# geopolars/geopolars

Measured on AMD Instinct MI355X. Metric: predicate evals/sec (10M pts x 1k polys point-in-polygon), higher is better.
Workload: dtype f64

## Files before the change

geopolars_amd/_abi.py:

```python
from __future__ import annotations

import ctypes as C
import os

HERE = os.path.dirname(os.path.abspath(__file__))
LIB_PATH = os.environ.get("GPK_LIB_PATH") or os.path.join(HERE, "libgeopolars_hip.so")

GPK_OK = 0
GPK_ERR_MISMATCHED_GEOMETRY = 1
GPK_ERR_INVALID_OFFSETS = 2
GPK_ERR_NULL_UNSUPPORTED = 3
GPK_ERR_DEVICE = 4
GPK_ERR_OOM = 5
GPK_ERR_INVALID_ARGUMENT = 6
GPK_ERR_CAPACITY = 7

GEOM_POINT = 0
GEOM_LINESTRING = 1
GEOM_POLYGON = 3
GEOM_MULTIPOINT = 4
GEOM_MULTILINESTRING = 5
GEOM_MULTIPOLYGON = 6
ARROW_WKB, ARROW_INTERLEAVED, ARROW_STRUCT = 0, 1, 2

# ... 101 lines not shown
    "gpk_envelope": (C.c_int32, [_VP, _VP, _VP, C.c_int32, _VP]),
    "gpk_exterior": (C.c_int32, [_VP, _VP, _VP, C.POINTER(C.c_int64), C.c_int32, _VP]),
    "gpk_explode": (C.c_int32, [_VP, _VP, C.c_int32, _VP, C.POINTER(_VP)]),
    "gpk_geoarray_validity": (C.c_int32, [_VP, _VP, C.POINTER(C.c_int32), _VP]),
    "gpk_geoarray_len": (C.c_int32, [_VP, C.POINTER(C.c_int64)]),
    "gpk_geom_type": (C.c_int32, [_VP, _VP, C.c_int32, _VP]),
    "gpk_is_empty": (C.c_int32, [_VP, _VP, C.c_int32, _VP]),
    "gpk_is_ring": (C.c_int32, [_VP, _VP, C.c_int32, _VP]),
    "gpk_point_xy": (C.c_int32, [_VP, _VP, _VP, C.c_int32, _VP]),
    "gpk_geodesic_length": (C.c_int32, [_VP, C.c_int32, _VP, C.c_int32, _VP]),
    "gpk_simplify": (C.c_int32, [_VP, C.c_double, _VP, _VP, C.POINTER(C.c_int64), C.c_int32, _VP]),
    "gpk_convex_hull": (C.c_int32, [_VP, _VP, _VP, C.c_int32, _VP]),
    "gpk_distance_rowwise": (C.c_int32, [_VP, _VP, _VP, _VP, C.c_int32, _VP]),
    "gpk_rowmap_build": (C.c_int32, [_VP, _VP, C.c_int64, C.c_int32, _VP, C.POINTER(_VP)]),
    "gpk_rowmap_free": (C.c_int32, [_VP]),
    "gpk_rowmap_nbytes": (C.c_int32, [_VP, C.POINTER(C.c_int64)]),
    "gpk_distance_rowmap": (C.c_int32, [_VP, _VP, _VP, _VP, C.c_int32, _VP]),
    "gpk_predicate_rowwise": (C.c_int32, [_VP, _VP, _VP, C.c_int32, _VP, C.c_int32, _VP]),
    "gpk_index_build": (C.c_int32, [_VP, _VP, C.POINTER(_VP)]),
    "gpk_index_build_ex": (C.c_int32, [_VP, C.c_int32, _VP, _VP, C.POINTER(_VP)]),
    "gpk_index_free": (C.c_int32, [_VP]),
    "gpk_index_nbytes": (C.c_int32, [_VP, C.POINTER(C.c_int64)]),
    "gpk_index_describe": (C.c_int32, [_VP, C.POINTER(C.c_int64)]),
    "gpk_index_query_envelope": (C.c_int32, [_VP, _VP, C.c_int64, C.c_int32, _VP, _VP, C.c_int64, C.POINTER(C.c_int64), C.c_int32, _VP]),
    "gpk_spatial_join": (
        C.c_int32,
        [_VP, _VP, _VP, C.c_int32, C.c_uint32, _VP, _VP, C.c_int64, C.POINTER(C.c_int64), C.c_int32, _VP],
    ),
    "gpk_spatial_join_async": (C.c_int32, [_VP, _VP, _VP, C.c_int32, C.c_uint32, _VP, _VP, C.c_int64, _VP, _VP]),
    "gpk_nearest_join": (
        C.c_int32,
        [_VP, _VP, _VP, C.c_double, C.c_uint32, _VP, _VP, _VP, C.c_int64, C.POINTER(C.c_int64), C.c_int32, _VP],
    ),
    "gpk_dwithin_join": (
        C.c_int32,
        [_VP, _VP, _VP, C.c_double, C.c_uint32, _VP, _VP, _VP, C.c_int64, C.POINTER(C.c_int64), C.c_int32, _VP],
    ),
    "gpk_dwithin_rowwise": (C.c_int32, [_VP, _VP, _VP, C.c_double, _VP, C.c_int32, _VP]),
    "gpk_closest_point_rowwise": (C.c_int32, [_VP, _VP, _VP, _VP, _VP, C.c_int32, _VP]),
    "gpk_line_locate_point": (C.c_int32, [_VP, _VP, _VP, C.c_int32, _VP, C.c_int32, _VP]),
    "gpk_line_interpolate_point": (C.c_int32, [_VP, _VP, C.c_int64, C.c_int32, _VP, _VP, C.c_int32, _VP]),
    "gpk_wkb_encode": (C.c_int32, [_VP, _VP, _VP, C.c_int64, C.POINTER(C.c_int64)]),
    "gpk_geoarray_to_wkb": (C.c_int32, [_VP, _VP, _VP, C.c_int64, C.POINTER(C.c_int64), C.c_int32, _VP]),
    "gpk_join_indices": (C.c_int32, [_VP, _VP, C.c_int64, C.c_int64, C.c_uint32, C.c_int32, _VP, _VP, C.c_int64, C.POINTER(C.c_int64), C.c_int32, _VP]),
    "gpk_take_fixed": (C.c_int32, [_VP, C.c_int32, _VP, C.c_int64, _VP, C.c_int64, _VP, _VP, C.c_int32, _VP]),
    "gpk_take_binary": (C.c_int32, [_VP, _VP, _VP, C.c_int64, _VP, C.c_int64, _VP, _VP, C.c_int64, C.POINTER(C.c_int64), _VP, C.c_int32, _VP]),
# ... 73 lines not shown
```

geopolars_amd/csrc/gpk_gridindex.hip:

```cpp
#include <atomic>
#include <chrono>
#include <cmath>
#include <cstdlib>

#include "gpk_device.h"
#include "gpk_index.h"
#include "gpk_scan.h"

namespace gpk {

__global__ __launch_bounds__(256) void extent_partial_kernel(const double4* __restrict__ bbox, int64_t n, double4* __restrict__ part) {
    __shared__ double red[4][4];
    double mnx = INFINITY, mny = INFINITY, mxx = -INFINITY, mxy = -INFINITY;
    for (int64_t i = (int64_t)blockIdx.x * 256 + threadIdx.x; i < n; i += (int64_t)gridDim.x * 256) {
        const double4 b = bbox[i];
        if (b.x == b.x) {
            mnx = fmin(mnx, b.x);
            mny = fmin(mny, b.y);
            mxx = fmax(mxx, b.z);
            mxy = fmax(mxy, b.w);
        }
    }
    mnx = dev::wave_min(mnx);
    mny = dev::wave_min(mny);
// ... 108 lines not shown
extern "C" {

int32_t gpk_index_free(gpk_index* idx) {
    if (!idx) return GPK_OK;
    int cur = -1;
    (void)hipGetDevice(&cur);
    if (cur != idx->device) (void)hipSetDevice(idx->device);
    (void)hipDeviceSynchronize();
    for (int i = 0; i < 24; ++i)
        if (idx->owned[i]) cached_free(idx->owned[i]);
    if (cur >= 0 && cur != idx->device) (void)hipSetDevice(cur);
    delete idx;
    return GPK_OK;
}

int32_t gpk_index_describe(const gpk_index* idx, int64_t out[8]) {
    if (!idx || !out) return fail(GPK_ERR_INVALID_ARGUMENT, "NULL argument");
    for (int i = 0; i < 8; ++i) out[i] = 0;
    out[0] = idx->pip.R;
    out[1] = idx->pip_lean;
    out[2] = idx->pip.chain_xy != nullptr;
    out[3] = idx->pip.route != nullptr;
    out[4] = idx->pip_list_heavy;
    return GPK_OK;
}

int32_t gpk_index_nbytes(const gpk_index* idx, int64_t* out_bytes) {
    if (!idx || !out_bytes) return fail(GPK_ERR_INVALID_ARGUMENT, "NULL argument");
    *out_bytes = idx->nbytes;
    return GPK_OK;
}

int32_t gpk_index_build(const gpk_geoarray* a, void* stream, gpk_index** out) {
    return gpk_index_build_ex(a, GPK_INDEX_BBOX_GRID | GPK_INDEX_PIP, nullptr, stream, out);
}

int32_t gpk_index_build_ex(const gpk_geoarray* a, int32_t parts, const double* bbox4_dev, void* stream, gpk_index** out) {
    if (!a || !out) return fail(GPK_ERR_INVALID_ARGUMENT, "NULL argument");
    *out = nullptr;
    GPK_TRY(require_device());
    hipStream_t s = (hipStream_t)stream;
    const int64_t n = a->d.n_geoms;

    gpk_index* ix = new gpk_index;
    memset(ix, 0, sizeof *ix);
    ix->device = a->device;
// ... 115 lines not shown
```

geopolars_amd/csrc/gpk_index.h:

```cpp
#pragma once

#include "gpk_common.h"

namespace gpk {

struct GridParams {
    double x0, y0, inv_w, inv_h;
    int32_t gx, gy;
};

struct IndexView {
    const double4* bbox;
    const GridParams* grid;
    const int32_t* cell_off;
    const int32_t* items;
    int32_t gx, gy;
};

struct PartInfo {
    int32_t slab_base, row0 , nrows, n_rings;
};
constexpr int PIP_SUB = 8;
constexpr int PIP_SLAB_MUL = 2;
constexpr int PIP_FINE_LOG2 = 6;
// ... 4 lines not shown
    uint32_t part_flags;
    uint32_t e0, e1, e2;
    uint32_t labels[4];
};
struct SubCell2 {
    SubCell a;
    uint32_t b_part_flags;
    uint32_t b_e0, b_e1, b_e2;
    uint32_t pad[4];
};
constexpr uint32_t SUB2_BIT = 1u << 29;
constexpr int CHAIN_MAX = 12;
constexpr uint32_t HCHAIN_COUNT_MASK = 0xFu;
constexpr int HCHAIN_BASE_SHIFT = 4;
constexpr int HCHAIN_START_SHIFT = 8;
struct HalfCell {
    uint32_t lw[2];
    uint32_t part_flags;
    uint32_t aux_base;
};
static_assert(sizeof(HalfCell) * 2 == sizeof(SubCell), "two half-cell records overlay one SubCell");
static_assert(CHAIN_MAX <= (int)HCHAIN_COUNT_MASK, "the edge count of a chain is a 4-bit field");
constexpr int PIP_ROUTE_RMAX = 512;
struct RouteWord {
    uint32_t bmask;
    uint32_t gmask;
    uint32_t rec0;
    uint32_t pad;
};
struct PipView {
    int32_t R;
    double rx0, ry0, fw, fh, inv_fw, inv_fh;
    const uint32_t* cell;
    const uint32_t* list;
    const SubCell* sub;
    const SubCell2* sub2;
    const double2* chain_xy;
    const RouteWord* route;
    const SubCell* lrec;
    const uint32_t* part_geom;
    const PartInfo* part_info;
    const float4* part_box;
    const int32_t* ring_row0;
    const int32_t* ring_slab_base;
    const int32_t* slab_off;
    const double4* slab_edges;
    const int32_t* slab_vidx;
    const double2* slab_xy;
};
constexpr uint32_t CELL_TAG_EMPTY = 0u, CELL_TAG_SINGLE = 1u, CELL_TAG_LIST = 2u, CELL_TAG_SUB = 3u;

namespace dev {
__device__ __forceinline__ int cell_of(double v, double v0, double inv, int g) {
    return (int)fmin(fmax((v - v0) * inv, 0.0), (double)(g - 1));
}
}

}

struct gpk_index {
    gpk::IndexView v;
// ... 18 lines not shown
```

geopolars_amd/csrc/gpk_join.hip:

```cpp
#include <cstdlib>
#include <cstring>
#include <mutex>
#include <type_traits>

#include <rocprim/rocprim.hpp>

#include "gpk_device.h"
#include "gpk_index.h"
#include "gpk_candjoin.h"
#include "gpk_pip.h"
#include "gpk_scan.h"
#include "gpk_pipshared.h"

namespace gpk {

constexpr int PIP_BLOCK = 256;
constexpr int WR_BLOCK = 256;
constexpr int PIP_PPT = 2;
constexpr int PIP_TILE = PIP_BLOCK * PIP_PPT;
constexpr int PIP_GS = 8;
constexpr int PIP_OVF = 256;
constexpr int PIP_QCAP = PIP_BLOCK * PIP_PPT;
constexpr int PIP_SUPER_SHIFT = 6;
constexpr int PIP_WPT = 8;
// ... 1255 lines not shown
    (void)hipGetDevice(&dev);
    if (dev >= 0 && dev < 16) {
        g_fused[dev].last = s;
        g_fused[dev].any = true;
        if (!launched) g_fused[dev].n = 0;
    }
    g_fused_mu.unlock();
}

static int32_t pip_join_enqueue(const gpk_geoarray* left, const gpk_geoarray* right, const gpk_index* right_index, uint32_t left_row_base,
                                uint32_t* out_counts, uint32_t* out_pairs, int64_t pair_capacity, bool host_out,
                                unsigned long long* total_out, hipStream_t s, uint32_t** counts_dev_out, uint32_t** pairs_dev_out,
                                unsigned long long** grand_out) {
    const int64_t n = left->d.n_geoms;
    const bool lean = right_index->pip.R > 0 && right_index->pip_lean;
    static const bool no_flow = [] {
        const char* e = getenv("GPK_TILE_KERNEL");
        return e && !strcmp(e, "chain");
    }();
    PipView pvj = right_index->pip;
    pvj.slab_xy = right->d.xy;
    const bool chain = right_index->pip.R > 0 && right_index->pip.chain_xy != nullptr;
    const bool one_per_lane = !chain && !lean && right_index->pip.R > 0 && right_index->pip_list_heavy;
    const int flow_p = chain && !no_flow && right_index->pip.route != nullptr && right_index->pip.R <= PIP_ROUTE_RMAX
                           ? pip_flow_points_per_lane(n, right->d.n_geoms, right_index->pip.R, cu_count())
                           : 0;
    const bool flow = flow_p > 0;
    const int tile_points = flow ? 64 * flow_p : (chain ? 64 * CHAIN_PPT : (lean ? LEAN_TILE : (one_per_lane ? PIP_BLOCK : PIP_TILE)));
    const int64_t n_blocks = (n + tile_points - 1) / tile_points;
    const bool want_pairs = pair_capacity > 0;
    const size_t counts_bytes = sizeof(uint32_t) * (size_t)n;
    const size_t pairs_bytes = sizeof(uint32_t) * 2 * (size_t)pair_capacity;
    const int64_t n_super = (n_blocks >> PIP_SUPER_SHIFT) + 1;
    const int64_t n_wblocks = (n + PIP_WTILE - 1) / PIP_WTILE;
    const uint32_t multi_cap = chain ? 1024u : (uint32_t)(n < (int64_t)0x18000000 ? 2 * n + 1024 : (int64_t)0x30000000);
    int64_t flow_wgs = (int64_t)cu_count();
    {
        const int64_t want = (n_blocks + 15) / 16;
        if (flow_wgs > want) flow_wgs = want;
        if (flow_wgs < 1) flow_wgs = 1;
    }
    const bool fused = flow;
    const size_t stage_bytes = flow ? pip_flow_pool_bytes(n) : 0;
    size_t need = align256(fused ? 64 : counts_bytes + 64)  + align256(sizeof(unsigned long long) * (size_t)(n_blocks + n_super + 3)) +
                  align256(sizeof(uint32_t) * (size_t)multi_cap) + align256(sizeof(ChainCold)) + align256(stage_bytes) + 1024;
    if (host_out && out_counts) need += align256(counts_bytes);
    if (host_out && want_pairs) need += align256(pairs_bytes);
// ... 33 lines not shown
        if (me != hipSuccess) return fail(GPK_ERR_DEVICE, "spatial_join: %s", hipGetErrorString(me));
    }
    ChainHot hot;
    memset(&hot, 0, sizeof hot);
    if (chain) {
        const PipView& pv = right_index->pip;
        hot.pts_xy = left->d.xy;
        hot.pts_validity = left->d.validity;
        hot.n_points = n;
        hot.n_tiles = n_blocks;
        hot.polys_validity = right->d.validity;
        hot.R = pv.R;
        hot.logR = 0;
        while ((1 << hot.logR) < pv.R) ++hot.logR;
        hot.rx0 = pv.rx0;
        hot.ry0 = pv.ry0;
        hot.inv_fw = pv.inv_fw;
        hot.inv_fh = pv.inv_fh;
        hot.cell = pv.cell;
        hot.half = reinterpret_cast<const HalfCell*>(pv.sub);
        hot.chain_xy = pv.chain_xy;
        hot.part_geom = pv.part_geom;
        hot.route = pv.route;
        hot.counts = counts_dev;
        hot.code = code;
        hot.block_tot = btot;
        hot.super_tot = stot;
        hot.stats = stats;
        hot.cold = cold;
        hot.stage = nullptr;
        hot.pool = reinterpret_cast<uint32_t*>(stage);
        hot.n_full_tiles = left->d.validity ? 0 : (int32_t)(n / tile_points);
        hot.inv_fw_s = pv.inv_fw * (double)PIP_SUB;
        hot.inv_fh_s = pv.inv_fh * (double)PIP_SUB;
        hot.sub_max = (double)(((uint32_t)PIP_SUB << hot.logR) - 1u);
    }
    if (flow) {
        const int64_t wgs = flow_wgs;
        FusedTail tail;
        memset(&tail, 0, sizeof tail);
        tail.pairs = (uint2*)pairs_dev;
        tail.capacity = pair_capacity;
        tail.grand = grand;
        tail.grand_host = total_out;
        tail.left_base = left_row_base;
        FusedWords fw;
// ... 279 lines not shown
```

geopolars_amd/csrc/gpk_pipflow.hip:

```cpp
#include "gpk_pipshared.h"

namespace gpk {

constexpr int FLOW_P_MAX = 8;
constexpr int FLOW_BLOCK = 1024, FLOW_W = FLOW_BLOCK / 64;
constexpr int FLOW_ITEMS = 128;
constexpr int FLOW_PASS_AT = 40;
constexpr int FLOW_MAX_TILES = 1536;
constexpr int FLOW_ID_BITS = 22;
constexpr uint32_t FLOW_DEAD = 0xFFFFFFFFu;
constexpr uint32_t FLOW_MULTI = 0x80000000u;
constexpr uint32_t FLOW_PEND = FLOW_MULTI;
static_assert(64 * FLOW_P_MAX == 512, "an entry keeps the row within its tile in 9 bits");
static_assert(FLOW_MAX_TILES <= (1 << 14), "FlowItem::loc keeps the tile in 14 bits");

struct FlowItem {
    double px, py;
    uint32_t aux;
    uint32_t loc;
};
static_assert(sizeof(FlowItem) == 24, "list slot");

#ifdef GPK_TILE_TRACE
#define FLOW_STAMP(i)                                                                                                    \
// ... 152 lines not shown
            const uint32_t li = (uint32_t)__shfl((int)e, j, 64) & 511u, row = (tile << ts) + li, slot = i + (uint32_t)j;
            const double2 q = pts_xy[row];
            const unsigned long long cf = chain_generic_row_first_call(cold, q.x, q.y, lane);
            const uint32_t cnt = (uint32_t)cf, first = (uint32_t)(cf >> 32);
            if (lane == 0) {
                if (stats) atomicAdd(&stats[2], 1ull);
                if (cnt == 0u) {
                    seg[slot] = FLOW_DEAD;
                    if (counts) counts[row] = 0u;
                    atomicSub(&s_ttot[t], 1u);
                } else if (cnt == 1u) {
                    seg[slot] = (first << 9) | li;
                } else {
                    seg[slot] = FLOW_MULTI | (cnt << 9) | li;
                    if (counts) counts[row] = cnt;
                    atomicAdd(&s_ttot[t], cnt - 1u);
                }
            }
        }
    }
}

template <bool SIMPLE, bool FULL, int P>
__device__ __forceinline__ void flow_tile(const ChainHot& h, const uint2* s_mask, const uint32_t* s_rec0, FlowItem* items, uint32_t& n_list, uint32_t t,
                                          uint32_t tile0, int lane, uint32_t* s_tcand, uint32_t* s_ttot FLOW_PHASE_ARGS) {
    constexpr int S = PIP_SUB, FLOW_TILE = 64 * P, TS = P == 8 ? 9 : (P == 4 ? 8 : (P == 2 ? 7 : 6));
    static_assert(P == 1 || P == 2 || P == 4 || P == 8, "tile sizes");
    static_assert(S == 8, "the sub-cell arithmetic below is written for 8 x 8 sub-cells");
    asm volatile("" : "+v"(lane));
    const uint32_t tile = tile0 + t;
    const int64_t base = (int64_t)tile * FLOW_TILE;
    const int64_t n_points = FULL ? 0 : H_COLD(n_points);
    const uint32_t rem = FULL ? (uint32_t)FLOW_TILE : (uint32_t)(n_points - base < (int64_t)FLOW_TILE ? n_points - base : (int64_t)FLOW_TILE);
    double px[P], py[P];
    {
        const double2* __restrict__ tile_xy = h.pts_xy + base;
        static_for<P>([&](auto K) {
            constexpr int k = decltype(K)::value;
            double2 v = make_double2(NAN, NAN);
            if (FULL || ((uint32_t)(k * 64 + lane) < rem && dev::valid_row(H_COLD(pts_validity), base + k * 64 + lane))) v = dev::load_stream(tile_xy + (k * 64 + lane));
            px[k] = v.x;
            py[k] = v.y;
        });
    }
    GPK_SCHED_FENCE();
    FLOW_PHASE(1);
    const int logR = h.logR;
    const uint32_t sub_max = ((uint32_t)S << logR) - 1u;
    uint32_t sidx4[(P + 3) / 4], gw[P];
    u32x4 rec[P];
    static_for<(P + 3) / 4>([&](auto J) { sidx4[decltype(J)::value] = 0u; });
    uint32_t sxs[P], sys_[P], r0s[P];
    uint2 ms[P];
    static_for<P>([&](auto K) {
        constexpr int k = decltype(K)::value;
        uint32_t sx = cvt_u32_sat((px[k] - h.rx0) * h.inv_fw_s), sy = cvt_u32_sat((py[k] - h.ry0) * h.inv_fh_s);
        sx = sx < sub_max ? sx : sub_max;
        sy = sy < sub_max ? sy : sub_max;
        const uint32_t at = ((sy >> 3) << (logR - 5)) + (sx >> 8);
        ms[k] = s_mask[at];
        r0s[k] = s_rec0[at];
        sxs[k] = sx;
        sys_[k] = sy;
    });
    GPK_SCHED_FENCE();
    static_for<P>([&](auto K) {
        constexpr int k = decltype(K)::value;
        const uint32_t sx = sxs[k], sy = sys_[k], bit = (sx >> 3) & 31u;
        const bool real = !__builtin_isunordered(px[k], py[k]);
        const bool has = real && ((ms[k].x >> bit) & 1u) != 0u;
        const bool want = real && !has && ((ms[k].y >> bit) & 1u) != 0u;
        sidx4[k / 4] |= (((sy & 3u) << 3) | (sx & 7u)) << (8 * (k % 4));
        rec[k] = u32x4{0u, 0u, 0u, 0u};
        gw[k] = 0u;
        if (has) {
            const uint32_t w = r0s[k] + (uint32_t)__popc(__builtin_amdgcn_ubfe(ms[k].x, 0u, bit));
            rec[k] = *reinterpret_cast<const u32x4*>(h.half + (2u * w + ((sy >> 2) & 1u)));
        }
        if (want) gw[k] = h.cell[((sy >> 3) << logR) + (sx >> 3)];
    });
    GPK_SCHED_FENCE();
    FLOW_PHASE(2);
    uint32_t run = 0u, n_new = 0u;
    bool pend = false;
    uint32_t* const tile_counts = h.counts ? h.counts + base : nullptr;
    uint32_t* const tile_pool = h.pool + ((size_t)tile << TS);
    static_for<P>([&](auto K) {
        constexpr int k = decltype(K)::value;
        const uint32_t li = (uint32_t)(k * 64 + lane);
        const uint32_t s5 = (sidx4[k / 4] >> (8 * (k % 4))) & 31u;
        const uint32_t lw = (s5 & 16u) ? rec[k].y : rec[k].x;
        const uint32_t lab = (lw >> (2u * (s5 & 15u))) & 3u;
        uint32_t r = lab ? (rec[k].z & 0x3FFFFFFFu) : CODE_NONE;
        const uint32_t g = gw[k];
        const bool single = (g & 0xC0000001u) == 0x40000000u;
        if (single) r = (g >> 1) & 0x1FFFFFFFu;
        const bool walk = g != 0u && !single;
        if (!SIMPLE) {
            if (r != CODE_NONE) {
                const uint32_t geom = h.part_geom ? h.part_geom[r] : r;
                r = dev::valid_row(h.polys_validity, geom) ? geom : CODE_NONE;
            }
// ... 10 lines not shown
            if (__builtin_expect(n_list + n_new + (uint32_t)__popcll(ml) > (uint32_t)FLOW_ITEMS, 0)) {
                if (listed && n_list + n_new + lanes_below(ml) >= (uint32_t)FLOW_ITEMS) {
                    listed = false;
                    e = FLOW_PEND | li;
                }
                ml = __ballot(listed);
                pend = true;
            }
            if (listed) {
                FlowItem* it = items + (n_list + n_new + lanes_below(ml));
                it->px = px[k];
                it->py = py[k];
                it->aux = walk ? 0u : rec[k].w;
                it->loc = (t << 18) | (rank << 9) | li;
            }
            n_new += (uint32_t)__popcll(ml);
        }
        if (tile_counts && mine) dev::store_stream(tile_counts + li, cand ? 1u : 0u);
        if (cand) tile_pool[rank] = e;
        run += (uint32_t)__popcll(mcand);
        GPK_SCHED_FENCE();
    });
    if (lane == 0) {
        s_tcand[t] = run;
        s_ttot[t] = run;
    }
    n_list += n_new;
    FLOW_PHASE(3);
    if (__builtin_expect(pend, 0)) flow_settle_pending(h.pts_xy, H_COLD(cold), h.pool, h.counts, H_COLD(stats), s_ttot, t, tile, run, lane, TS);
}

__device__ __forceinline__ void flow_emit_chunk(const ChainHot& h, uint32_t e, uint32_t row0, uint32_t pt0, unsigned long long* out64, uint32_t room, uint32_t& done,
                                                int lane) {
    const bool live = e != FLOW_DEAD;
    const bool multi = live && (e & FLOW_MULTI) != 0u;
    const unsigned long long mm = __ballot(multi);
    if (__builtin_expect(mm == 0ull, 1)) {
        const unsigned long long m = __ballot(live);
        const uint32_t at = done + lanes_below(m);
        if (live && at < room) __builtin_nontemporal_store(((unsigned long long)(e >> 9) << 32) | (unsigned long long)(row0 + (e & 511u)), out64 + at);
        done += (uint32_t)__popcll(m);
        return;
    }
    const uint32_t n_out = !live ? 0u : (multi ? (e >> 9) & ((1u << FLOW_ID_BITS) - 1u) : 1u);
    uint32_t incl = n_out;
#pragma unroll
    for (int o = 1; o < 64; o <<= 1) {
        const uint32_t v = __shfl_up(incl, o, 64);
        if (lane >= o) incl += v;
    }
    const uint32_t at = done + incl - n_out;
    if (live && !multi && at < room) __builtin_nontemporal_store(((unsigned long long)(e >> 9) << 32) | (unsigned long long)(row0 + (e & 511u)), out64 + at);
    unsigned long long wm = mm;
    while (wm) {
        const int j = __builtin_ctzll(wm);
        wm &= wm - 1ull;
        const uint32_t lj = (uint32_t)__shfl((int)e, j, 64) & 511u, aj = (uint32_t)__shfl((int)at, j, 64);
        const double2 q = h.pts_xy[pt0 + lj];
        chain_generic_row_call(H_COLD(cold), q.x, q.y, lane, reinterpret_cast<uint2*>(out64 + aj), aj < room ? room - aj : 0u, row0 + lj);
    }
    done += (uint32_t)__shfl((int)incl, 63, 64);
}

template <bool SIMPLE, int P>
__global__ __launch_bounds__(FLOW_BLOCK) void pip_tile_flow_kernel(ChainHot h, FusedTail tail) {
    constexpr int WORDS = PIP_ROUTE_RMAX * PIP_ROUTE_RMAX / 32, W = FLOW_W, TS = P == 8 ? 9 : (P == 4 ? 8 : (P == 2 ? 7 : 6));
    __shared__ uint2 s_mask[WORDS];
    __shared__ uint32_t s_rec0[WORDS];
    __shared__ FlowItem s_items[W][FLOW_ITEMS];
    __shared__ uint32_t s_tcand[FLOW_MAX_TILES], s_ttot[FLOW_MAX_TILES];
    __shared__ uint32_t s_next, s_next2, s_wg, s_wgtot, s_gave_up;
    __shared__ unsigned long long s_part[W];
    const int lane = threadIdx.x & 63, wave = __builtin_amdgcn_readfirstlane(threadIdx.x >> 6);
    FLOW_STAMP(0);
    unsigned long long my_ticket = 0ull;
    if (threadIdx.x == 0) my_ticket = __hip_atomic_fetch_add(T_COLD(ticket), 1ull, __ATOMIC_RELAXED, __HIP_MEMORY_SCOPE_AGENT);
    {
        const int R = H_COLD(R), words = R * R / 32;
        const uint4* __restrict__ src = reinterpret_cast<const uint4*>(H_COLD(route));
        for (int i = threadIdx.x; i < words; i += FLOW_BLOCK) {
            const uint4 rw = src[i];
            s_mask[i] = make_uint2(rw.x, rw.y);
            s_rec0[i] = rw.z;
        }
    }
    FLOW_STAMP(1);
    if (threadIdx.x == 0) {
        s_wg = (uint32_t)(my_ticket - T_COLD(ticket_base));
        s_next = 0u;
        s_next2 = 0u;
        s_gave_up = 0u;
    }
    __syncthreads();
    const uint32_t wg = __builtin_amdgcn_readfirstlane(s_wg);
    const uint32_t T0 = (uint32_t)((int64_t)wg * H_COLD(n_tiles) / (int64_t)gridDim.x), T1 = (uint32_t)((int64_t)(wg + 1u) * H_COLD(n_tiles) / (int64_t)gridDim.x);
    const uint32_t nt = T1 - T0;
    const bool want_pairs = T_COLD(pairs) != nullptr;
    FLOW_STAMP(2);
    const uint32_t nf = (int64_t)T1 <= (int64_t)H_COLD(n_full_tiles) ? nt : ((int64_t)T0 >= (int64_t)H_COLD(n_full_tiles) ? 0u : (uint32_t)(H_COLD(n_full_tiles) - (int32_t)T0));
    uint32_t n_list = 0u;
#ifdef GPK_TILE_TRACE
    int n_mine = 0;
#if GPK_TILE_TRACE == 2
    unsigned long long g_phase[6] = {0ull, 0ull, 0ull, 0ull, 0ull, 0ull}, g_last = wall_clock64();
#endif
#endif
    auto draw = [&](uint32_t* counter) -> uint32_t {
        __builtin_amdgcn_wave_barrier();
        const uint32_t d = __hip_atomic_fetch_add(counter, 1u, __ATOMIC_RELAXED, __HIP_MEMORY_SCOPE_WORKGROUP);
        return __builtin_amdgcn_readfirstlane(d) >> 6;
    };
    {
        uint32_t t = draw(&s_next);
        while (t < nf) {
            const uint32_t tn = draw(&s_next);
            FLOW_PHASE(4);
            if (n_list >= (uint32_t)FLOW_PASS_AT) flow_exact_pass<TS>(h, s_items[wave], n_list, lane, s_ttot, T0);
            FLOW_PHASE(0);
            flow_tile<SIMPLE, true, P>(h, s_mask, s_rec0, s_items[wave], n_list, t, T0, lane, s_tcand, s_ttot FLOW_PHASE_PASS);
            t = tn;
#if defined(GPK_TILE_TRACE) && GPK_TILE_TRACE != 2
            if (n_mine < 6) FLOW_STAMP(3 + n_mine);
            ++n_mine;
#endif
        }
    }
    for (;;) {
        const uint32_t t = draw(&s_next2) + nf;
        if (t >= nt) break;
        if (n_list >= (uint32_t)FLOW_PASS_AT) flow_exact_pass<TS>(h, s_items[wave], n_list, lane, s_ttot, T0);
        flow_tile<SIMPLE, false, P>(h, s_mask, s_rec0, s_items[wave], n_list, t, T0, lane, s_tcand, s_ttot FLOW_PHASE_PASS);
    }
    while (n_list) flow_exact_pass<TS>(h, s_items[wave], n_list, lane, s_ttot, T0);
#if defined(GPK_TILE_TRACE) && GPK_TILE_TRACE == 2
    FLOW_PHASE(5);
    if (h.stats && lane == 0 && wave % 5 == 0 && blockIdx.x < 900u)
        for (int i = 0; i < 6; ++i) h.stats[8 + (blockIdx.x * 4 + wave / 5) * 16 + 3 + i] = g_phase[i];
#endif
    FLOW_STAMP(9);
    __syncthreads();
    FLOW_STAMP(10);
    constexpr int EM_C = P < 4 ? P : 4, EM_T = 24 / EM_C;
    uint32_t ent[EM_T][EM_C], cand[EM_T];
    auto em_request = [&](uint32_t first) {
        static_for<EM_T>([&](auto Rr) {
            constexpr int r = decltype(Rr)::value;
            const uint32_t et = first + (uint32_t)(r * W);
            cand[r] = et < nt && want_pairs ? s_tcand[et] : 0u;
            cand[r] = __builtin_amdgcn_readfirstlane(cand[r]);
            const uint32_t* seg = h.pool + ((size_t)(T0 + et) << TS);
            static_for<EM_C>([&](auto Cc) {
                constexpr int c = decltype(Cc)::value;
                ent[r][c] = FLOW_DEAD;
                if ((uint32_t)(c * 64 + lane) < cand[r]) ent[r][c] = seg[c * 64 + lane];
// ... 127 lines not shown
```

geopolars_amd/csrc/gpk_pipindex.hip:

```cpp
#include <cstdio>
#include <cstdlib>
#include <cstring>

#include <rocprim/rocprim.hpp>

#include <chrono>

#include "gpk_device.h"
#include "gpk_index.h"
#include "gpk_pip.h"
#include "gpk_scan.h"

namespace gpk {

struct FineGrid {
    int R;
    double rx0, ry0, fw, fh, inv_fw, inv_fh, pad_x, pad_y;
};
__device__ __forceinline__ int fcol(const FineGrid& f, double x) { return dev::cell_of(x, f.rx0, f.inv_fw, f.R); }
__device__ __forceinline__ int frow(const FineGrid& f, double y) { return dev::cell_of(y, f.ry0, f.inv_fh, f.R); }

__global__ void part_geom_kernel(DevGeo a, uint32_t* __restrict__ part_geom) {
    const int64_t g = (int64_t)blockIdx.x * blockDim.x + threadIdx.x;
    if (g >= a.n_geoms) return;
// ... 714 lines not shown
    h[1] = HalfCell{{rc.labels[2], rc.labels[3]}, rc.part_flags & ~SUB_INDIRECT, hword[2 * i + 1]};
}
__global__ void route_build_kernel(const uint32_t* __restrict__ cell, int64_t n_words, RouteWord* __restrict__ route) {
    const int64_t w = (int64_t)blockIdx.x * blockDim.x + threadIdx.x;
    if (w >= n_words) return;
    RouteWord rw{0u, 0u, 0u, 0u};
    bool have = false;
    for (int i = 0; i < 32; ++i) {
        const uint32_t cw = cell[32 * w + i];
        const uint32_t tag = cw >> 30, payload = cw & 0x3FFFFFFFu;
        if (tag == CELL_TAG_SUB && !(payload & SUB2_BIT)) {
            rw.bmask |= 1u << i;
            if (!have) {
                rw.rec0 = payload;
                have = true;
            }
        } else if (cw != 0u) {
            rw.gmask |= 1u << i;
        }
    }
    route[w] = rw;
}

__global__ void route_rank_kernel(RouteWord* __restrict__ route, int R) {
    const int row = blockIdx.x * blockDim.x + threadIdx.x;
    if (row >= R) return;
    const int per_row = R / 32;
    RouteWord* rw = route + (int64_t)row * per_row;
    uint32_t base = 0u;
    bool have = false;
    for (int j = 0; j < per_row; ++j) {
        if (rw[j].bmask && !have) {
            base = rw[j].rec0;
            have = true;
        }
        rw[j].pad = rw[j].bmask ? rw[j].rec0 - base : 0u;
    }
}

__global__ void sub_work_kernel(const uint32_t* __restrict__ cell, const int32_t* __restrict__ flag, const int32_t* __restrict__ pos,
                                int64_t n_cells, int32_t* __restrict__ work_cell, uint32_t* __restrict__ work_part) {
    const int64_t c = (int64_t)blockIdx.x * blockDim.x + threadIdx.x;
    if (c >= n_cells || !flag[c]) return;
    work_cell[pos[c]] = (int32_t)c;
    work_part[pos[c]] = (cell[c] & 0x3FFFFFFFu) >> 1;
}
__global__ void lrec_assign_kernel(const uint32_t* __restrict__ cell, uint32_t* __restrict__ list, int64_t n_cells,
                                   const int32_t* __restrict__ pos, int32_t* __restrict__ work_cell, uint32_t* __restrict__ work_part) {
    const int64_t c = (int64_t)blockIdx.x * blockDim.x + threadIdx.x;
    if (c >= n_cells) return;
    const uint32_t w = cell[c];
    if ((w >> 30) != CELL_TAG_LIST) return;
    const uint32_t off = w & 0x3FFFFFFFu, m = list[off];
    int32_t o = pos[c];
    for (uint32_t t = 0; t < m; ++t) {
        const uint32_t e = list[off + 1 + t];
        if (!(e & 1u)) continue;
        work_cell[o] = (int32_t)c;
        work_part[o] = e >> 1;
        list[off + 1 + t] = ((uint32_t)o << 1) | 1u;
// ... 395 lines not shown
    const bool boundary_cells_have_records = level2_ok && !sub_overflow && n_sub2 == 0;
    ix->pip_lean = (int64_t)list_len * 8 <= (int64_t)n_sub && n_refined == 0 && boundary_cells_have_records ? 1 : 0;
    if (getenv("GPK_DEBUG_INDEX")) fprintf(stderr, "[gpk] lean join kernel eligible: %d (list %d, refined rings: %s, one-part records %d)\n", ix->pip_lean, list_len, n_refined ? "some" : "none", n_sub);
    if (ix->pip_lean && slab_vidx && n_sub > 0 && swork_cell && d.n_coords + d.n_rings * CHAIN_MAX < ((int64_t)1 << (32 - HCHAIN_START_SHIFT))) {
        const int64_t n_ext = d.n_coords + d.n_rings * CHAIN_MAX;
        double2* cxy = nullptr;
        GPK_HIP(cached_malloc((void**)&cxy, sizeof(double2) * (size_t)n_ext));
        keep(cxy);
        uint32_t* hword;
        GPK_TRY(t.alloc(&hword, (size_t)n_sub * 2 + 2));
        pv.sub = sub;
        GPK_LAUNCH("gpk_pipidx_chain_xy", chain_xy_kernel, blocks_for(n_ext), dim3(256), 0, s, d, cxy);
        GPK_LAUNCH("gpk_pipidx_half_chain", half_chain_kernel, blocks_for((int64_t)n_sub * 2), dim3(256), 0, s, d, pv, g,
                   (const int32_t*)swork_cell, (const uint32_t*)swork_part, (int64_t)n_sub, (const int32_t*)slab_vidx, (const SubCell*)sub, hword);
        GPK_LAUNCH("gpk_pipidx_chain_commit", half_chain_commit_kernel, blocks_for(n_sub), dim3(256), 0, s, sub, (int64_t)n_sub, (const uint32_t*)hword);
        pv.chain_xy = cxy;
        ix->nbytes += (int64_t)(sizeof(double2) * (size_t)n_ext);
        if (R <= PIP_ROUTE_RMAX) {
            RouteWord* route = nullptr;
            const int64_t n_words = n_cells / 32;
            GPK_HIP(cached_malloc((void**)&route, sizeof(RouteWord) * (size_t)n_words));
            keep(route);
            GPK_LAUNCH("gpk_pipidx_route", route_build_kernel, blocks_for(n_words), dim3(256), 0, s, (const uint32_t*)cell, n_words, route);
            if (R >= 32) GPK_LAUNCH("gpk_pipidx_route_rank", route_rank_kernel, dim3((unsigned)((R + 63) / 64)), dim3(64), 0, s, route, R);
            pv.route = route;
            ix->nbytes += (int64_t)(sizeof(RouteWord) * (size_t)n_words);
        }
        GPK_HIP(hipStreamSynchronize(s));
        if (getenv("GPK_DEBUG_INDEX")) fprintf(stderr, "[gpk] half-cell chains: %d records, %lld extended coordinates%s\n", n_sub, (long long)n_ext, pv.route ? ", routing image" : "");
        stamp("local chains");
    }
    ix->nbytes += (int64_t)(sizeof(SubCell) * (size_t)n_sub + sizeof(SubCell2) * (size_t)n_sub2 + sizeof(SubCell) * (size_t)n_lrec);
    ix->pip = pv;
    ix->nbytes += (int64_t)(sizeof(uint32_t) * (size_t)n_cells + sizeof(uint32_t) * (size_t)list_len + (pv.slab_edges ? sizeof(double4) : sizeof(int32_t)) * (size_t)n_edges +
                            sizeof(int32_t) * (size_t)(n_slabs + 1) + sizeof(int32_t) * (size_t)(2 * n_rings + 1) +
                            (part_geom ? sizeof(uint32_t) * (size_t)n_parts : 0) + sizeof(PartInfo) * (size_t)n_parts);
    return GPK_OK;
}

}
```

geopolars_amd/csrc/gpk_pipshared.h:

```cpp
#pragma once

#include <type_traits>

#include "gpk_device.h"
#include "gpk_index.h"

namespace gpk {

constexpr uint32_t CODE_NONE = 0xFFFFFFFFu, CODE_MULTI = 0xFFFFFFFEu;
constexpr uint32_t CODE_POOL = 0x80000000u;

#define GPK_SCHED_FENCE() __builtin_amdgcn_sched_barrier(0)
template <int N, typename F>
__device__ __forceinline__ void static_for(F&& f) {
    if constexpr (N > 0) {
        static_for<N - 1>(f);
        f(std::integral_constant<int, N - 1>{});
    }
}

struct ChainHot {
    const double2* pts_xy;
    const uint8_t* pts_validity;
    int64_t n_points, n_tiles;
    const uint8_t* polys_validity;
    int32_t R, logR;
    double rx0, ry0, inv_fw, inv_fh;
    const uint32_t* cell;
    const HalfCell* half;
    const double2* chain_xy;
    const uint32_t* part_geom;
    const RouteWord* route;
    uint32_t* counts;
    uint32_t* code;
    unsigned long long* block_tot;
    unsigned long long* super_tot;
    unsigned long long* stats;
    const struct ChainCold* cold;
    uint2* stage;
    int32_t n_full_tiles, pad;
    double inv_fw_s, inv_fh_s, sub_max;
    uint32_t* pool;
};
struct ChainCold {
    DevGeo polys;
    IndexView ix;
    GridParams grid;
};

template <bool INLINE_EXACT>
__device__ __forceinline__ uint32_t chain_generic_row(const ChainCold* __restrict__ cold, double px, double py, int lane, uint32_t* first,
                                                      uint2* emit = nullptr, uint32_t emit_room = 0u, uint32_t l = 0u) {
    const DevGeo polys = cold->polys;
    const IndexView ix = cold->ix;
    const GridParams g = cold->grid;
    uint32_t cnt = 0;
    *first = CODE_NONE;
    if (!(px == px && py == py)) return 0u;
    const int cx = dev::cell_of(px, g.x0, g.inv_w, g.gx), cy = dev::cell_of(py, g.y0, g.inv_h, g.gy);
    const int cc = cy * g.gx + cx;
    for (int q = ix.cell_off[cc]; q < ix.cell_off[cc + 1]; ++q) {
        const int j = ix.items[q];
        const double4 bb = ix.bbox[j];
        if (!(px >= bb.x && px <= bb.z && py >= bb.y && py <= bb.w) || !dev::valid_row(polys.validity, j)) continue;
        int p0, p1;
// ... 90 lines not shown
```

include/geopolars_hip.h:

```cpp
#ifndef GEOPOLARS_HIP_H
#define GEOPOLARS_HIP_H

#include <stddef.h>
#include <stdint.h>

#ifdef __cplusplus
extern "C" {
#endif

#define GPK_OK                        0
#define GPK_ERR_MISMATCHED_GEOMETRY   1
#define GPK_ERR_INVALID_OFFSETS       2
#define GPK_ERR_NULL_UNSUPPORTED      3
#define GPK_ERR_DEVICE                4
#define GPK_ERR_OOM                   5
#define GPK_ERR_INVALID_ARGUMENT      6
#define GPK_ERR_CAPACITY              7

#define GPK_GEOM_POINT             0
#define GPK_GEOM_LINESTRING        1
#define GPK_GEOM_POLYGON           3
#define GPK_GEOM_MULTIPOINT        4
#define GPK_GEOM_MULTILINESTRING   5
#define GPK_GEOM_MULTIPOLYGON      6
// ... 126 lines not shown
                         void* stream, gpk_rowmap** out);
int32_t gpk_rowmap_free(gpk_rowmap* map);
int32_t gpk_rowmap_nbytes(const gpk_rowmap* map, int64_t* out_bytes);
int32_t gpk_distance_rowmap(const gpk_geoarray* a, const gpk_geoarray* b, const gpk_rowmap* map, double* out,
                            int32_t out_space, void* stream);
int32_t gpk_predicate_rowwise(const gpk_geoarray* a, const gpk_geoarray* b, const uint32_t* b_rows,
                              int32_t predicate, uint8_t* out, int32_t out_space, void* stream);

int32_t gpk_index_build(const gpk_geoarray* a, void* stream, gpk_index** out);
#define GPK_INDEX_BBOX_GRID 1
#define GPK_INDEX_PIP       2
#define GPK_INDEX_PIP_LIGHT 4
#define GPK_INDEX_PIP_FULL  8
int32_t gpk_index_build_ex(const gpk_geoarray* a, int32_t parts, const double* bbox4_dev, void* stream,
                           gpk_index** out);
int32_t gpk_index_free(gpk_index* idx);
#define GPK_QUERY_CONTAINED    0
#define GPK_QUERY_INTERSECTING 1
int32_t gpk_index_query_envelope(const gpk_index* idx, const double* boxes4, int64_t n_boxes, int32_t mode,
                                 uint32_t* out_counts, uint32_t* out_pairs, int64_t pair_capacity, int64_t* n_pairs,
                                 int32_t space, void* stream);
int32_t gpk_index_nbytes(const gpk_index* idx, int64_t* out_bytes);
int32_t gpk_index_describe(const gpk_index* idx, int64_t out[8]);

int32_t gpk_spatial_join(const gpk_geoarray* left, const gpk_geoarray* right,
                         const gpk_index* right_index, int32_t predicate, uint32_t left_row_base,
                         uint32_t* out_counts, uint32_t* out_pairs, int64_t pair_capacity,
                         int64_t* n_pairs, int32_t out_space, void* stream);

int32_t gpk_nearest_join(const gpk_geoarray* left, const gpk_geoarray* right, const gpk_index* right_index, double max_distance,
                         uint32_t left_row_base, uint32_t* out_counts, uint32_t* out_pairs, double* out_dist, int64_t pair_capacity,
                         int64_t* n_pairs, int32_t out_space, void* stream);

int32_t gpk_dwithin_join(const gpk_geoarray* left, const gpk_geoarray* right, const gpk_index* right_index, double distance,
                         uint32_t left_row_base, uint32_t* out_counts, uint32_t* out_pairs, double* out_dist, int64_t pair_capacity,
                         int64_t* n_pairs, int32_t out_space, void* stream);
int32_t gpk_dwithin_rowwise(const gpk_geoarray* a, const gpk_geoarray* b, const uint32_t* b_rows, double distance, uint8_t* out,
                            int32_t out_space, void* stream);

int32_t gpk_closest_point_rowwise(const gpk_geoarray* a, const gpk_geoarray* b, const uint32_t* b_rows, double* out_xy, int32_t* out_seg,
                                  int32_t out_space, void* stream);
int32_t gpk_line_locate_point(const gpk_geoarray* pts, const gpk_geoarray* lines, const uint32_t* line_rows, int32_t normalized, double* out,
                              int32_t out_space, void* stream);
int32_t gpk_line_interpolate_point(const gpk_geoarray* lines, const double* distances, int64_t n_distances, int32_t normalized,
                                   double* out_xy, uint8_t* out_valid, int32_t out_space, void* stream);

// ... 46 lines not shown
```

Measured before the change: 112700 billion.

## Compact per-cell words into ranked gword array with per-row bases for PIP flow

Replaces the direct cell[] lookup in the PIP flow tile with a compacted gword array indexed by a rank computed from the routing bitmasks, stored as 16-bit in-row ranks plus per-row base offsets kept in shared memory. The aim is for the per-point cell-word fetch to touch a dense array of only the relevant words, which should make the gathers more cache-friendly. It also narrows s_tcand to 16 bits and adds an index-build pass, a single-block prefix scan and a debug export API for the route image. The trade-offs are more shared memory, a longer index build, and 16-bit rank fields that require R to stay at or below 512.

```diff
diff --git a/geopolars_amd/_abi.py b/geopolars_amd/_abi.py
--- a/geopolars_amd/_abi.py
+++ b/geopolars_amd/_abi.py
@@ -147,6 +147,7 @@
     "gpk_index_free": (C.c_int32, [_VP]),
     "gpk_index_nbytes": (C.c_int32, [_VP, C.POINTER(C.c_int64)]),
     "gpk_index_describe": (C.c_int32, [_VP, C.POINTER(C.c_int64)]),
+    "gpk_index_route_image": (C.c_int32, [_VP, C.POINTER(C.c_double), _VP, C.c_int64, C.POINTER(C.c_int64), _VP]),
     "gpk_index_query_envelope": (C.c_int32, [_VP, _VP, C.c_int64, C.c_int32, _VP, _VP, C.c_int64, C.POINTER(C.c_int64), C.c_int32, _VP]),
     "gpk_spatial_join": (
         C.c_int32,
diff --git a/geopolars_amd/csrc/gpk_gridindex.hip b/geopolars_amd/csrc/gpk_gridindex.hip
--- a/geopolars_amd/csrc/gpk_gridindex.hip
+++ b/geopolars_amd/csrc/gpk_gridindex.hip
@@ -154,6 +154,27 @@
     out[2] = idx->pip.chain_xy != nullptr;
     out[3] = idx->pip.route != nullptr;
     out[4] = idx->pip_list_heavy;
+    return GPK_OK;
+}
+
+int32_t gpk_index_route_image(const gpk_index* idx, double geom[4], uint32_t* words, int64_t capacity, int64_t* n_words, void* stream) {
+    if (!idx || !n_words) return fail(GPK_ERR_INVALID_ARGUMENT, "NULL argument");
+    const gpk::PipView& pv = idx->pip;
+    const bool have = pv.route != nullptr && pv.route_row != nullptr && pv.R >= 32;
+    *n_words = have ? (int64_t)pv.R * pv.R / 32 * 4 + 2 * (int64_t)pv.R : 0;
+    if (geom) {
+        geom[0] = pv.rx0;
+        geom[1] = pv.ry0;
+        geom[2] = pv.fw;
+        geom[3] = pv.fh;
+    }
+    if (!have || !words) return GPK_OK;
+    if (capacity < *n_words) return fail(GPK_ERR_CAPACITY, "index_route_image: %lld words, room for %lld", (long long)*n_words, (long long)capacity);
+    hipStream_t s = (hipStream_t)stream;
+    const size_t image = sizeof(gpk::RouteWord) * (size_t)pv.R * (size_t)pv.R / 32;
+    GPK_HIP(hipMemcpyAsync(words, pv.route, image, hipMemcpyDeviceToHost, s));
+    GPK_HIP(hipMemcpyAsync(words + image / 4, pv.route_row, sizeof(uint2) * (size_t)pv.R, hipMemcpyDeviceToHost, s));
+    GPK_HIP(hipStreamSynchronize(s));
     return GPK_OK;
 }
 
diff --git a/geopolars_amd/csrc/gpk_index.h b/geopolars_amd/csrc/gpk_index.h
--- a/geopolars_amd/csrc/gpk_index.h
+++ b/geopolars_amd/csrc/gpk_index.h
@@ -50,11 +50,12 @@
 static_assert(sizeof(HalfCell) * 2 == sizeof(SubCell), "two half-cell records overlay one SubCell");
 static_assert(CHAIN_MAX <= (int)HCHAIN_COUNT_MASK, "the edge count of a chain is a 4-bit field");
 constexpr int PIP_ROUTE_RMAX = 512;
+static_assert(PIP_ROUTE_RMAX <= 0xFFFF, "in-row ranks of records and of level-1 words are 16-bit fields");
 struct RouteWord {
     uint32_t bmask;
     uint32_t gmask;
     uint32_t rec0;
-    uint32_t pad;
+    uint32_t rank;
 };
 struct PipView {
     int32_t R;
@@ -65,6 +66,8 @@
     const SubCell2* sub2;
     const double2* chain_xy;
     const RouteWord* route;
+    const uint32_t* gword;
+    const uint2* route_row;
     const SubCell* lrec;
     const uint32_t* part_geom;
     const PartInfo* part_info;
diff --git a/geopolars_amd/csrc/gpk_join.hip b/geopolars_amd/csrc/gpk_join.hip
--- a/geopolars_amd/csrc/gpk_join.hip
+++ b/geopolars_amd/csrc/gpk_join.hip
@@ -1301,7 +1301,7 @@
     pvj.slab_xy = right->d.xy;
     const bool chain = right_index->pip.R > 0 && right_index->pip.chain_xy != nullptr;
     const bool one_per_lane = !chain && !lean && right_index->pip.R > 0 && right_index->pip_list_heavy;
-    const int flow_p = chain && !no_flow && right_index->pip.route != nullptr && right_index->pip.R <= PIP_ROUTE_RMAX
+    const int flow_p = chain && !no_flow && right_index->pip.route != nullptr && right_index->pip.gword != nullptr && right_index->pip.R <= PIP_ROUTE_RMAX
                            ? pip_flow_points_per_lane(n, right->d.n_geoms, right_index->pip.R, cu_count())
                            : 0;
     const bool flow = flow_p > 0;
@@ -1381,6 +1381,8 @@
         hot.chain_xy = pv.chain_xy;
         hot.part_geom = pv.part_geom;
         hot.route = pv.route;
+        hot.gword = pv.gword;
+        hot.route_row = pv.route_row;
         hot.counts = counts_dev;
         hot.code = code;
         hot.block_tot = btot;
diff --git a/geopolars_amd/csrc/gpk_pipflow.hip b/geopolars_amd/csrc/gpk_pipflow.hip
--- a/geopolars_amd/csrc/gpk_pipflow.hip
+++ b/geopolars_amd/csrc/gpk_pipflow.hip
@@ -198,8 +198,8 @@
 }
 
 template <bool SIMPLE, bool FULL, int P>
-__device__ __forceinline__ void flow_tile(const ChainHot& h, const uint2* s_mask, const uint32_t* s_rec0, FlowItem* items, uint32_t& n_list, uint32_t t,
-                                          uint32_t tile0, int lane, uint32_t* s_tcand, uint32_t* s_ttot FLOW_PHASE_ARGS) {
+__device__ __forceinline__ void flow_tile(const ChainHot& h, const uint2* s_mask, const uint32_t* s_rank, const uint2* s_row, FlowItem* items, uint32_t& n_list,
+                                          uint32_t t, uint32_t tile0, int lane, uint16_t* s_tcand, uint32_t* s_ttot FLOW_PHASE_ARGS) {
     constexpr int S = PIP_SUB, FLOW_TILE = 64 * P, TS = P == 8 ? 9 : (P == 4 ? 8 : (P == 2 ? 7 : 6));
     static_assert(P == 1 || P == 2 || P == 4 || P == 8, "tile sizes");
     static_assert(S == 8, "the sub-cell arithmetic below is written for 8 x 8 sub-cells");
@@ -226,8 +226,8 @@
     uint32_t sidx4[(P + 3) / 4], gw[P];
     u32x4 rec[P];
     static_for<(P + 3) / 4>([&](auto J) { sidx4[decltype(J)::value] = 0u; });
-    uint32_t sxs[P], sys_[P], r0s[P];
-    uint2 ms[P];
+    uint32_t sxs[P], sys_[P], rks[P];
+    uint2 ms[P], rbs[P];
     static_for<P>([&](auto K) {
         constexpr int k = decltype(K)::value;
         uint32_t sx = cvt_u32_sat((px[k] - h.rx0) * h.inv_fw_s), sy = cvt_u32_sat((py[k] - h.ry0) * h.inv_fh_s);
@@ -235,7 +235,8 @@
         sy = sy < sub_max ? sy : sub_max;
         const uint32_t at = ((sy >> 3) << (logR - 5)) + (sx >> 8);
         ms[k] = s_mask[at];
-        r0s[k] = s_rec0[at];
+        rks[k] = s_rank[at];
+        rbs[k] = s_row[sy >> 3];
         sxs[k] = sx;
         sys_[k] = sy;
     });
@@ -249,11 +250,9 @@
         sidx4[k / 4] |= (((sy & 3u) << 3) | (sx & 7u)) << (8 * (k % 4));
         rec[k] = u32x4{0u, 0u, 0u, 0u};
         gw[k] = 0u;
-        if (has) {
-            const uint32_t w = r0s[k] + (uint32_t)__popc(__builtin_amdgcn_ubfe(ms[k].x, 0u, bit));
-            rec[k] = *reinterpret_cast<const u32x4*>(h.half + (2u * w + ((sy >> 2) & 1u)));
-        }
-        if (want) gw[k] = h.cell[((sy >> 3) << logR) + (sx >> 3)];
+        const uint32_t w = (has ? rbs[k].x + (rks[k] & 0xFFFFu) : rbs[k].y + (rks[k] >> 16)) + (uint32_t)__popc(__builtin_amdgcn_ubfe(has ? ms[k].x : ms[k].y, 0u, bit));
+        if (has) rec[k] = *reinterpret_cast<const u32x4*>(h.half + (2u * w + ((sy >> 2) & 1u)));
+        if (want) gw[k] = h.gword[w];
     });
     GPK_SCHED_FENCE();
     FLOW_PHASE(2);
@@ -310,7 +309,7 @@
         GPK_SCHED_FENCE();
     });
     if (lane == 0) {
-        s_tcand[t] = run;
+        s_tcand[t] = (uint16_t)run;
         s_ttot[t] = run;
     }
     n_list += n_new;
@@ -354,9 +353,11 @@
 __global__ __launch_bounds__(FLOW_BLOCK) void pip_tile_flow_kernel(ChainHot h, FusedTail tail) {
     constexpr int WORDS = PIP_ROUTE_RMAX * PIP_ROUTE_RMAX / 32, W = FLOW_W, TS = P == 8 ? 9 : (P == 4 ? 8 : (P == 2 ? 7 : 6));
     __shared__ uint2 s_mask[WORDS];
-    __shared__ uint32_t s_rec0[WORDS];
+    __shared__ uint32_t s_rank[WORDS];
+    __shared__ uint2 s_row[PIP_ROUTE_RMAX];
     __shared__ FlowItem s_items[W][FLOW_ITEMS];
-    __shared__ uint32_t s_tcand[FLOW_MAX_TILES], s_ttot[FLOW_MAX_TILES];
+    __shared__ uint16_t s_tcand[FLOW_MAX_TILES];
+    __shared__ uint32_t s_ttot[FLOW_MAX_TILES];
     __shared__ uint32_t s_next, s_next2, s_wg, s_wgtot, s_gave_up;
     __shared__ unsigned long long s_part[W];
     const int lane = threadIdx.x & 63, wave = __builtin_amdgcn_readfirstlane(threadIdx.x >> 6);
@@ -369,8 +370,10 @@
         for (int i = threadIdx.x; i < words; i += FLOW_BLOCK) {
             const uint4 rw = src[i];
             s_mask[i] = make_uint2(rw.x, rw.y);
-            s_rec0[i] = rw.z;
-        }
+            s_rank[i] = rw.w;
+        }
+        const uint2* __restrict__ rows = H_COLD(route_row);
+        for (int i = threadIdx.x; i < R; i += FLOW_BLOCK) s_row[i] = rows[i];
     }
     FLOW_STAMP(1);
     if (threadIdx.x == 0) {
@@ -405,7 +408,7 @@
             FLOW_PHASE(4);
             if (n_list >= (uint32_t)FLOW_PASS_AT) flow_exact_pass<TS>(h, s_items[wave], n_list, lane, s_ttot, T0);
             FLOW_PHASE(0);
-            flow_tile<SIMPLE, true, P>(h, s_mask, s_rec0, s_items[wave], n_list, t, T0, lane, s_tcand, s_ttot FLOW_PHASE_PASS);
+            flow_tile<SIMPLE, true, P>(h, s_mask, s_rank, s_row, s_items[wave], n_list, t, T0, lane, s_tcand, s_ttot FLOW_PHASE_PASS);
             t = tn;
 #if defined(GPK_TILE_TRACE) && GPK_TILE_TRACE != 2
             if (n_mine < 6) FLOW_STAMP(3 + n_mine);
@@ -417,7 +420,7 @@
         const uint32_t t = draw(&s_next2) + nf;
         if (t >= nt) break;
         if (n_list >= (uint32_t)FLOW_PASS_AT) flow_exact_pass<TS>(h, s_items[wave], n_list, lane, s_ttot, T0);
-        flow_tile<SIMPLE, false, P>(h, s_mask, s_rec0, s_items[wave], n_list, t, T0, lane, s_tcand, s_ttot FLOW_PHASE_PASS);
+        flow_tile<SIMPLE, false, P>(h, s_mask, s_rank, s_row, s_items[wave], n_list, t, T0, lane, s_tcand, s_ttot FLOW_PHASE_PASS);
     }
     while (n_list) flow_exact_pass<TS>(h, s_items[wave], n_list, lane, s_ttot, T0);
 #if defined(GPK_TILE_TRACE) && GPK_TILE_TRACE == 2
diff --git a/geopolars_amd/csrc/gpk_pipindex.hip b/geopolars_amd/csrc/gpk_pipindex.hip
--- a/geopolars_amd/csrc/gpk_pipindex.hip
+++ b/geopolars_amd/csrc/gpk_pipindex.hip
@@ -760,20 +760,35 @@
     route[w] = rw;
 }
 
-__global__ void route_rank_kernel(RouteWord* __restrict__ route, int R) {
-    const int row = blockIdx.x * blockDim.x + threadIdx.x;
-    if (row >= R) return;
+__global__ __launch_bounds__(PIP_ROUTE_RMAX) void route_rank_kernel(RouteWord* __restrict__ route, int R, uint2* __restrict__ row_base) {
+    __shared__ uint32_t s_cnt[PIP_ROUTE_RMAX];
+    const int row = threadIdx.x;
     const int per_row = R / 32;
     RouteWord* rw = route + (int64_t)row * per_row;
-    uint32_t base = 0u;
+    uint32_t base = 0u, g = 0u;
     bool have = false;
     for (int j = 0; j < per_row; ++j) {
-        if (rw[j].bmask && !have) {
-            base = rw[j].rec0;
+        const RouteWord w = rw[j];
+        if (w.bmask && !have) {
+            base = w.rec0;
             have = true;
         }
-        rw[j].pad = rw[j].bmask ? rw[j].rec0 - base : 0u;
-    }
+        rw[j].rank = (w.bmask ? w.rec0 - base : 0u) | (g << 16);
+        g += (uint32_t)__popc(w.gmask);
+    }
+    s_cnt[row] = g;
+    __syncthreads();
+    uint32_t before = 0u;
+    for (int i = 0; i < row; ++i) before += s_cnt[i];
+    row_base[row] = make_uint2(base, before);
+}
+__global__ void route_gword_kernel(const uint32_t* __restrict__ cell, const RouteWord* __restrict__ route, const uint2* __restrict__ row_base,
+                                   int64_t n_words, int per_row, uint32_t* __restrict__ gword) {
+    const int64_t w = (int64_t)blockIdx.x * blockDim.x + threadIdx.x;
+    if (w >= n_words) return;
+    const RouteWord rw = route[w];
+    uint32_t at = row_base[w / per_row].y + (rw.rank >> 16);
+    for (uint32_t m = rw.gmask; m; m &= m - 1u) gword[at++] = cell[32 * w + __builtin_ctz(m)];
 }
 
 __global__ void sub_work_kernel(const uint32_t* __restrict__ cell, const int32_t* __restrict__ flag, const int32_t* __restrict__ pos,
@@ -1215,9 +1230,23 @@
             GPK_HIP(cached_malloc((void**)&route, sizeof(RouteWord) * (size_t)n_words));
             keep(route);
             GPK_LAUNCH("gpk_pipidx_route", route_build_kernel, blocks_for(n_words), dim3(256), 0, s, (const uint32_t*)cell, n_words, route);
-            if (R >= 32) GPK_LAUNCH("gpk_pipidx_route_rank", route_rank_kernel, dim3((unsigned)((R + 63) / 64)), dim3(64), 0, s, route, R);
             pv.route = route;
             ix->nbytes += (int64_t)(sizeof(RouteWord) * (size_t)n_words);
+            if (R >= 32) {
+                const size_t g_cap = (size_t)(n_cells - n_sub) + 1;
+                uint32_t* gword = nullptr;
+                uint2* route_row = nullptr;
+                GPK_HIP(cached_malloc((void**)&gword, sizeof(uint32_t) * g_cap));
+                keep(gword);
+                GPK_HIP(cached_malloc((void**)&route_row, sizeof(uint2) * (size_t)R));
+                keep(route_row);
+                GPK_LAUNCH("gpk_pipidx_route_rank", route_rank_kernel, dim3(1), dim3((unsigned)R), 0, s, route, R, route_row);
+                GPK_LAUNCH("gpk_pipidx_route_gword", route_gword_kernel, blocks_for(n_words), dim3(256), 0, s, (const uint32_t*)cell, (const RouteWord*)route,
+                           (const uint2*)route_row, n_words, R / 32, gword);
+                pv.gword = gword;
+                pv.route_row = route_row;
+                ix->nbytes += (int64_t)(sizeof(uint32_t) * g_cap + sizeof(uint2) * (size_t)R);
+            }
         }
         GPK_HIP(hipStreamSynchronize(s));
         if (getenv("GPK_DEBUG_INDEX")) fprintf(stderr, "[gpk] half-cell chains: %d records, %lld extended coordinates%s\n", n_sub, (long long)n_ext, pv.route ? ", routing image" : "");
diff --git a/geopolars_amd/csrc/gpk_pipshared.h b/geopolars_amd/csrc/gpk_pipshared.h
--- a/geopolars_amd/csrc/gpk_pipshared.h
+++ b/geopolars_amd/csrc/gpk_pipshared.h
@@ -41,6 +41,8 @@
     int32_t n_full_tiles, pad;
     double inv_fw_s, inv_fh_s, sub_max;
     uint32_t* pool;
+    const uint32_t* gword;
+    const uint2* route_row;
 };
 struct ChainCold {
     DevGeo polys;
diff --git a/include/geopolars_hip.h b/include/geopolars_hip.h
--- a/include/geopolars_hip.h
+++ b/include/geopolars_hip.h
@@ -172,6 +172,7 @@
                                  int32_t space, void* stream);
 int32_t gpk_index_nbytes(const gpk_index* idx, int64_t* out_bytes);
 int32_t gpk_index_describe(const gpk_index* idx, int64_t out[8]);
+int32_t gpk_index_route_image(const gpk_index* idx, double geom[4], uint32_t* words, int64_t capacity, int64_t* n_words, void* stream);
 
 int32_t gpk_spatial_join(const gpk_geoarray* left, const gpk_geoarray* right,
                          const gpk_index* right_index, int32_t predicate, uint32_t left_row_base,
```

Result: no change. 112200 billion (-0.4%).
